# fallenshock/SinDDM

Hardware: AMD Instinct MI355X
Metric: diffusion steps/sec (finest scale) + imgs/sec full multi-scale sample, 1/2/4/8 GPU (higher is better)
Workload: dtype f32 (3x3 convs: binary16 hi/lo split products -- Winograd-domain GEMMs with all 4 MFMA terms, fp32 accumulate; fp32-equivalent, error vs float64 = the fp32 oracle's: tests/test_gpu_h2.py; everything else fp32); 1 GPU; C3: 6-scale pyramid, T=1000, finest scale 411x512, batch 64 per GPU, dim=160; batch_per_gpu=64, global_batch=64, scale=5, parallelism=independent chains over 1 GPU(s), one all-gather of the images

## Files before the change

### include/sinddm_hip_debug.h

```cpp
#ifndef SINDDM_HIP_DEBUG_H
#define SINDDM_HIP_DEBUG_H

#include <stddef.h>
#include <stdint.h>

#ifdef __cplusplus
extern "C" {
#endif

int sinddm_prof_begin(void);
int sinddm_prof_end(double* conv_ms_total, int64_t* conv_launches, double* conv_flops_total);
int sinddm_prof_end2(double* conv_ms_total, int64_t* conv_launches, double* conv_flops_total,
                     double* conv_exec_flops_total);
int sinddm_prof_end3(int kind, double* ms_total, int64_t* launches, double* flops_total,
                     double* exec_flops_total, int reset);

int sinddm_debug_conv_path(int dim, int B, int H, int W);

int sinddm_debug_infer_path(int dim, int B, int H, int W);

int sinddm_debug_train_path(int dim, int B, int H, int W);

int sinddm_debug_block_train(const float* params, const float* packed, const float* packed_bwd, int dim, int l,
                             const float* x, const float* cond_bias, const float* grad_y, float* y, float* grad_x,
                             float* grad_params, float* dcond, int B, int H, int W, void* ws, size_t ws_bytes,
                             void* stream);

int sinddm_debug_wgrad_map(int Cin, int Cout, int64_t ntiles, int ncu, uint32_t* wg_out, int wg_cap, int32_t* splits_out,
                           int splits_cap);

#ifdef __cplusplus
}
#endif
#endif
```

### sinddm_amd/_lib.py

```python
from __future__ import annotations

import ctypes as C
import os
from typing import Optional

import torch

_HERE = os.path.dirname(os.path.abspath(__file__))
LIB_PATH = os.path.join(_HERE, "libsinddm_hip.so")

ABI_SYMBOLS = (
    "sinddm_abi_version", "sinddm_param_count", "sinddm_param_tensors", "sinddm_param_offset",
    "sinddm_packed_count", "sinddm_workspace_bytes", "sinddm_pack_weights", "sinddm_net_forward",
    "sinddm_q_sample", "sinddm_reverse_step", "sinddm_reverse_step_edit", "sinddm_upsample_bilinear", "sinddm_prof_begin", "sinddm_prof_end", "sinddm_prof_end2", "sinddm_prof_end3", "sinddm_debug_wgrad_map", "sinddm_debug_conv_path",
    "sinddm_debug_block_train", "sinddm_debug_infer_path", "sinddm_debug_train_path",
    "sinddm_train_workspace_bytes", "sinddm_packed_bwd_count", "sinddm_pack_weights_bwd",
    "sinddm_net_forward_train", "sinddm_net_backward", "sinddm_l1_loss_fwd_bwd", "sinddm_adam_ema_step",
    "sinddm_cond_embed", "sinddm_cond_stride", "sinddm_sample_chain", "sinddm_sample_chain2", "sinddm_sample_chain_ex",
    "sinddm_normal_fill", "sinddm_wrap_halo", "sinddm_upsample_bilinear_wrap", "sinddm_sample_chain_tile",
    "sinddm_sample_chain_keep", "sinddm_reverse_step_keep", "sinddm_normal_fill_samples", "sinddm_sample_chain_seeds",
)


ABI_VERSION = 3
DIM_FP32_CONVS = 0x10000
TILE_HALO = 16


class StepCoefs(C.Structure):
    _fields_ = [("mode", C.c_int), ("clip", C.c_int),
                ("sqrt_recip_ac_t", C.c_float), ("sqrt_recipm1_ac_t", C.c_float),
                ("coef1_t", C.c_float), ("coef2_t", C.c_float),
                ("gamma_t", C.c_float), ("gamma_tm1", C.c_float),
                ("sqrt_ac_tm1", C.c_float), ("sqrt_ac_t", C.c_float), ("sqrt_1m_ac_t", C.c_float),
                ("sqrt_1m_ac_tm1_mvar", C.c_float), ("sigma", C.c_float)]


class ChainOpts(C.Structure):
    _fields_ = [("edit_w", C.c_void_p), ("edit_c", C.c_void_p), ("noise", C.c_void_p)]


class KeepOpts(C.Structure):
    _fields_ = [("mask", C.c_void_p), ("x0", C.c_void_p), ("ab", C.POINTER(C.c_float))]


class SinddmError(RuntimeError):
    pass


_lib: Optional[C.CDLL] = None


def load() -> C.CDLL:
# ... 19 lines not shown
        "sinddm_param_tensors": (i, [i]),
        "sinddm_param_offset": (i64, [i, i]),
        "sinddm_packed_count": (i64, [i]),
        "sinddm_workspace_bytes": (sz, [i, i, i, i]),
        "sinddm_pack_weights": (i, [p, p, i, p]),
        "sinddm_net_forward": (i, [p, p, p, p, i, f, p, i, i, i, i, p, sz, p]),
        "sinddm_cond_embed": (i, [p, p, i, f, i, i, p, p, p, p]),
        "sinddm_cond_stride": (i, [i]),
        "sinddm_q_sample": (i, [p, p, p, p, p, p, p, p, i, i, i64, p]),
        "sinddm_reverse_step": (i, [p, p, p, p, p, C.POINTER(StepCoefs), i64, p]),
        "sinddm_reverse_step_edit": (i, [p, p, p, p, p, C.POINTER(StepCoefs), p, p, i, i, i, p]),
        "sinddm_sample_chain": (i, chain[:-2] + [C.POINTER(C.c_int)]),
        "sinddm_sample_chain2": (i, chain),
        "sinddm_sample_chain_ex": (i, chain + [C.POINTER(ChainOpts)]),
        "sinddm_sample_chain_tile": (i, chain + [C.POINTER(ChainOpts), i, i]),
        "sinddm_sample_chain_keep": (i, chain + [C.POINTER(ChainOpts), i, i, C.POINTER(KeepOpts)]),
        "sinddm_sample_chain_seeds": (i, chain + [C.POINTER(ChainOpts), i, i, C.POINTER(KeepOpts), p]),
        "sinddm_normal_fill_samples": (i, [p, i, i64, p, C.c_uint64, p]),
        "sinddm_reverse_step_keep": (i, [p, p, p, p, p, C.POINTER(StepCoefs), p, p, p, p, f, f, i, i, i, p]),
        "sinddm_wrap_halo": (i, [p, p, i, i, i, i, i, p]),
        "sinddm_upsample_bilinear_wrap": (i, [p, p, i, i, i, i, i, i, i, p]),
        "sinddm_normal_fill": (i, [p, i64, C.c_uint64, C.c_uint64, p]),
        "sinddm_upsample_bilinear": (i, [p, p, i, i, i, i, i, p]),
        "sinddm_prof_begin": (i, []),
        "sinddm_prof_end": (i, [C.POINTER(C.c_double), C.POINTER(C.c_int64), C.POINTER(C.c_double)]),
        "sinddm_prof_end2": (i, [C.POINTER(C.c_double), C.POINTER(C.c_int64), C.POINTER(C.c_double),
                                 C.POINTER(C.c_double)]),
        "sinddm_prof_end3": (i, [i, C.POINTER(C.c_double), C.POINTER(C.c_int64), C.POINTER(C.c_double),
                                 C.POINTER(C.c_double), i]),
        "sinddm_debug_wgrad_map": (i, [i, i, i64, i, C.POINTER(C.c_uint32), i, C.POINTER(C.c_int32), i]),
        "sinddm_debug_conv_path": (i, [i, i, i, i]),
        "sinddm_debug_infer_path": (i, [i, i, i, i]),
        "sinddm_debug_train_path": (i, [i, i, i, i]),
        "sinddm_debug_block_train": (i, [p, p, p, i, i, p, p, p, p, p, p, p, i, i, i, p, sz, p]),
        "sinddm_train_workspace_bytes": (sz, [i, i, i, i]),
        "sinddm_packed_bwd_count": (i64, [i]),
        "sinddm_pack_weights_bwd": (i, [p, p, i, p]),
        "sinddm_net_forward_train": (i, [p, p, p, p, i, f, p, i, i, i, i, p, sz, p]),
        "sinddm_net_backward": (i, [p, p, p, p, p, p, p, i, i, i, i, p, sz, p]),
        "sinddm_l1_loss_fwd_bwd": (i, [p, p, p, p, i64, f, p]),
        "sinddm_adam_ema_step": (i, [p, p, p, p, p, f, f, f, f, f, f, f, i, i64, p]),
    }
    for name, (res, args) in sig.items():
        if not hasattr(lib, name):
            continue
        fn = getattr(lib, name)
        fn.restype = res
        fn.argtypes = args
    _lib = lib
    return lib


def missing_symbols():
    lib = load()
    return [s for s in ABI_SYMBOLS if not hasattr(lib, s)]


def check(rc: int, what: str) -> None:
    if rc != 0:
        kind = {-1: "bad argument", -2: "unsupported shape", -3: "workspace too small"}.get(rc, f"hipError {rc}")
        raise SinddmError(f"{what} failed: {kind}")


def ptr(t: Optional[torch.Tensor]) -> Optional[int]:
    if t is None:
        return None
# ... 10 lines not shown
```

### sinddm_amd/csrc/internal.h

```cpp
#pragma once
#include "common.h"

namespace sinddm {

struct PackSeg {
    long long dst;
    long long count;
    long long w;
    long long w2;
    int kind;
    int cin, cout, taps, nch, mt, co_lds;
    int transpose;
};
struct PackArgs {
    PackSeg seg[32];
    int nseg;
    long long total;
};
int pack_launch(const float* params, float* packed, const PackArgs& a, hipStream_t st);

struct TrainBufs {
    float* cond;
    float* emb;
    float* hpre;
    float* cvec;
    float* mvec;
    float* h[4];
    float* u[4];
    float* g[4];
    float* o[4];
    float* s[4];
    float* dcond;
    float* small;
    float* wscr;
    float* amax;
};

struct ChainStep;
int net_forward_impl(const NetPlan& P, const float* params, const float* packed, const float* x, const int64_t* t_dev,
                     int t_host, float scale, float* out, int B, int H, int W, void* ws, size_t ws_bytes,
                     hipStream_t st, const TrainBufs* tb, const ChainStep* cs = nullptr);

int block_forward(const NetPlan& P, int l, const float* params, const float* packed, const float* cur, const float* cond,
                  int cond_stride, float* hbuf, float* gbuf, float* obuf, float* upre, int B, int H, int W, hipStream_t st,
                  int Wt = 0, float* amax = nullptr);
int conv3x3_path(int cout, int cin, int coblks, int B, int H, int W);

struct ConvArgs;
bool wh_applies(const NetPlan& P, int B, int H, int W, int cin, int cout);
bool wh_enabled();
int wh_conv(const ConvArgs& c, hipStream_t st);
int wh_pack(const float* w, float* wsinv, void* img, int cin, int cout, int transpose, hipStream_t st);
int amax_tensor_launch(const float* x, float* amax, int B, long long per_sample, hipStream_t st);

int dwconv_launch(const float* x, const float* w, const float* bias, const float* cond, int cond_stride,
                  const float* addt, int flip, float* out, int B, int C, int H, int W, hipStream_t st, int pi = 0, int po = 0,
                  float* amax = nullptr);

}
```

### sinddm_amd/csrc/plan.h

```cpp
#pragma once
#include <stdint.h>

namespace sinddm {

constexpr int KC = 8;
constexpr int TIME_DIM = 32;
constexpr int CHANNELS = 3;

inline bool wh_plan_ok(int cin, int cout) { return cin >= 32 && cin % 16 == 0 && cout % 80 == 0; }
inline long long wh_plan_halfs(int cin, int cout) { return (long long)(cout / 80) * (cin / 16) * 24 * 5 * 512; }

struct BlockPlan {
    int cin, cout;
    int64_t mlp_w, mlp_b, tr_w, tr_b, dw_w, dw_b, c1_w, c1_b, c2_w, c2_b, res_w, res_b;
    int mt;
    int coblks;
    int co_lds;
    int nch1;
    int nch2;
    int nchr;
    int64_t pk_c1, pk_c2, pk_res, pk_b1, pk_b2;
    int nchw1, nchw2;
    int64_t pk_wc1, pk_wc2;
    int64_t pk_w1f, pk_w2f;
    int64_t pk_q1, pk_q2, pk_qs1, pk_qs2;
    int cond_off;
};

struct NetPlan {
    int dim, half;
    BlockPlan blk[4];
    int64_t tm0_w, tm0_b, tm2_w, tm2_b, fin_w, fin_b;
    int64_t nparams, npacked;
    int64_t pk_zero;
    int ntensors;
    int64_t tensor_off[64];
    int cond_stride;
    bool fp32_convs;
    bool ok;
};

inline int mt_for(int cout) { return (cout % 80 == 0) ? 5 : ((cout % 32 == 0) ? 2 : 1); }
inline int co_lds_for(int mt) { int m = mt * 16; return (m % 32 == 16) ? m : m + 16; }

inline NetPlan make_plan(int dim_arg) {
    NetPlan p{};
    const int dim = dim_arg & 0xFFFF;
    p.fp32_convs = (dim_arg & 0x10000) != 0;
    if (dim_arg < 0 || (dim_arg >> 17) != 0) { p.ok = false; return p; }
    p.ok = dim >= 2 && dim % 2 == 0 && dim <= 1024;
    p.dim = dim;
    p.half = dim / 2;
    int64_t o = 0;
    int nt = 0;
    auto take = [&](int64_t n) { int64_t r = o; p.tensor_off[nt++] = r; o += n; return r; };
    p.tm0_w = take(TIME_DIM * 4 * TIME_DIM * 2);
    p.tm0_b = take(TIME_DIM * 4);
    p.tm2_w = take(TIME_DIM * TIME_DIM * 4);
    p.tm2_b = take(TIME_DIM);
    const int cins[4] = {CHANNELS, p.half, dim, dim};
    const int couts[4] = {p.half, dim, dim, p.half};
    int64_t q = 0;
    int coff = 0;
    for (int l = 0; l < 4; ++l) {
        BlockPlan& b = p.blk[l];
        b.cin = cins[l];
        b.cout = couts[l];
// ... 18 lines not shown
        b.co_lds = co_lds_for(b.mt);
        b.nch1 = (b.cin + KC - 1) / KC;
        b.nch2 = (b.cout + KC - 1) / KC;
        b.nchr = (b.res_w >= 0) ? (b.cin + KC - 1) / KC : 0;
        b.pk_c1 = q; q += (int64_t)b.coblks * b.nch1 * 9 * KC * b.co_lds;
        b.pk_c2 = q; q += (int64_t)b.coblks * b.nch2 * 9 * KC * b.co_lds;
        b.pk_res = q; q += (int64_t)b.coblks * b.nchr * KC * b.co_lds;
        b.pk_b1 = q; q += (int64_t)b.coblks * b.mt * 16;
        b.pk_b2 = q; q += (int64_t)b.coblks * b.mt * 16;
        b.nchw1 = (b.cin + 15) / 16;
        b.nchw2 = (b.cout + 15) / 16;
        if (b.cin >= 8) { b.pk_wc1 = q; q += (int64_t)b.coblks * b.nchw1 * 16 * 4 * b.mt * 64; } else b.pk_wc1 = -1;
        b.pk_wc2 = q; q += (int64_t)b.coblks * b.nchw2 * 16 * 4 * b.mt * 64;
        const bool f24 = b.mt == 5 && b.cout % 80 == 0;
        if (f24 && b.cin >= 16 && b.cin % 16 == 0) { b.pk_w1f = q; q += (int64_t)b.coblks * b.nchw1 * 32768; } else b.pk_w1f = -1;
        if (f24 && b.cout % 16 == 0) { b.pk_w2f = q; q += (int64_t)b.coblks * b.nchw2 * 32768; } else b.pk_w2f = -1;
        q = (q + 63) / 64 * 64;
        if (wh_plan_ok(b.cin, b.cout)) {
            b.pk_q1 = q; q += wh_plan_halfs(b.cin, b.cout) / 2;
            b.pk_qs1 = q; q += (b.cout + 63) / 64 * 64;
        } else b.pk_q1 = b.pk_qs1 = -1;
        if (wh_plan_ok(b.cout, b.cout)) {
            b.pk_q2 = q; q += wh_plan_halfs(b.cout, b.cout) / 2;
            b.pk_qs2 = q; q += (b.cout + 63) / 64 * 64;
        } else b.pk_q2 = b.pk_qs2 = -1;
        b.cond_off = coff;
        coff += b.cin;
    }
    p.fin_w = take((int64_t)CHANNELS * p.half);
    p.fin_b = take(CHANNELS);
    p.nparams = o;
    p.pk_zero = q;
    q += 64;
    p.npacked = q;
    p.ntensors = nt;
    p.cond_stride = (coff + 3) / 4 * 4;
    return p;
}

}
```

### sinddm_amd/csrc/sinddm_fwd.hip

```cpp
#include "conv_mfma.h"
#include "conv_wino.h"
#include "conv_wino4.h"
#include "conv_wh.h"
#include "internal.h"
#include "step_tail.h"
#include <type_traits>
namespace sinddm {

ConvProfiler& conv_profiler() {
    static ConvProfiler p;
    return p;
}

__global__ void pack_kernel(const float* __restrict__ params, float* __restrict__ packed, PackArgs a) {
    long long i = (long long)blockIdx.x * blockDim.x + threadIdx.x;
    if (i >= a.total) return;
    int s = 0;
    long long base = 0;
    while (s < a.nseg - 1 && i >= base + a.seg[s].count) { base += a.seg[s].count; ++s; }
    const PackSeg& g = a.seg[s];
    const long long j = i - base;
    float v = 0.0f;
    if (g.kind == 0) {
        const int co_l = (int)(j % g.co_lds);
// ... 154 lines not shown
    auto addf = [&](PackSeg sg) { f.seg[n++] = sg; total += sg.count; };
    for (int l = 0; l < 4; ++l) {
        const BlockPlan& b = P.blk[l];
        PackSeg wz{};
        wz.kind = 4; wz.mt = b.mt; wz.transpose = 0; wz.w2 = -1; wz.taps = 9;
        if (b.pk_w1f >= 0) {
            wz.dst = b.pk_w1f; wz.nch = b.nchw1; wz.count = (long long)b.coblks * b.nchw1 * 32768;
            wz.w = b.c1_w; wz.cin = b.cin; wz.cout = b.cout;
            addf(wz);
        }
        if (b.pk_w2f >= 0) {
            wz.dst = b.pk_w2f; wz.nch = b.nchw2; wz.count = (long long)b.coblks * b.nchw2 * 32768;
            wz.w = b.c2_w; wz.cin = b.cout; wz.cout = b.cout;
            addf(wz);
        }
    }
    if (n > 0) {
        f.nseg = n;
        f.total = total;
        rc = pack_launch(params, packed, f, st);
        if (rc) return rc;
    }
    for (int l = 0; l < 4; ++l) {
        const BlockPlan& b = P.blk[l];
        if (b.pk_q1 >= 0) {
            rc = wh_pack_launch(params + b.c1_w, packed + b.pk_qs1, packed + b.pk_q1, b.cin, b.cout, 0, st);
            if (rc) return rc;
        }
        if (b.pk_q2 >= 0) {
            rc = wh_pack_launch(params + b.c2_w, packed + b.pk_qs2, packed + b.pk_q2, b.cout, b.cout, 0, st);
            if (rc) return rc;
        }
    }
    return 0;
}

struct CondArgs {
    const float* params;
    const long long* t_dev;
    int t_host;
    int t_step;
    float scale;
    float* out;
    int cond_stride;
    long long tm0_w, tm0_b, tm2_w, tm2_b;
    long long mlp_w[4], mlp_b[4], tr_w[4], tr_b[4];
    int cin[4], coff[4];
    float* cond_vec;
    float* hidden;
    float* emb_out;
    float* mvec_out;
};
static CondArgs cond_args(const NetPlan& P, const float* params) {
    CondArgs ca{};
    ca.params = params; ca.cond_stride = P.cond_stride;
    ca.tm0_w = P.tm0_w; ca.tm0_b = P.tm0_b; ca.tm2_w = P.tm2_w; ca.tm2_b = P.tm2_b;
    for (int l = 0; l < 4; ++l) {
        ca.mlp_w[l] = P.blk[l].mlp_w; ca.mlp_b[l] = P.blk[l].mlp_b;
        ca.tr_w[l] = P.blk[l].tr_w; ca.tr_b[l] = P.blk[l].tr_b;
        ca.cin[l] = P.blk[l].cin; ca.coff[l] = P.blk[l].cond_off;
    }
    return ca;
}

__global__ __launch_bounds__(128) void cond_kernel(CondArgs a) {
    __shared__ float emb[64];
    __shared__ float h1[128];
// ... 526 lines not shown
    for (int l = 0; l < 4; ++l) {
        const BlockPlan& b = P.blk[l];
        if (b.cout % 4 != 0) return false;
        if (b.cin != 3 && !(b.pk_wc1 >= 0 && b.cin % 4 == 0)) return false;
    }
    return true;
}
static int fwd_pitch(const NetPlan& P, int W) { return (W % 4 != 0 && plan_pads_rows(P)) ? (W + 3) / 4 * 4 : W; }
static size_t fwd_xpad_bytes(const NetPlan& P, int B, int H, int W) {
    return fwd_pitch(P, W) != W ? align_up((size_t)B * CHANNELS * H * fwd_pitch(P, W) * sizeof(float), 256) : 0;
}
static size_t fwd_workspace_core(const NetPlan& P, int B, int H, int W) {
    const size_t act = align_up((size_t)B * P.dim * H * fwd_pitch(P, W) * sizeof(float), 256);
    return cond_region_bytes(P, B) + 4 * act + fwd_xpad_bytes(P, B, H, W);
}
static size_t fwd_workspace_bytes(const NetPlan& P, int B, int H, int W) {
    return fwd_workspace_core(P, B, H, W) + 2 * cond_region_bytes(P, (B + 1) / 2) + 4096;
}

struct ChainStep {
    const float* cond_row;
    const float* x_tilde;
    float* x_next;
    TailArgs tail;
};

template <class F>
static void tail_dispatch(const TailArgs& t, F&& f) {
    auto keep = [&](auto e, auto n) { t.km ? f(e, n, std::true_type{}) : f(e, n, std::false_type{}); };
    auto noise = [&](auto e) { t.nz ? keep(e, std::true_type{}) : keep(e, std::false_type{}); };
    t.ew ? noise(std::true_type{}) : noise(std::false_type{});
}

int conv3x3_path(int cout, int cin, int coblks, int B, int H, int W) {
    if (!wino_enabled() || cout % 4 != 0) return 0;
    const bool f24 = mt_for(cout) == 5 && cout % 80 == 0 && cin >= 16 && cin % 16 == 0;
    const bool v3 = SINDDM_WINO_V3 && f24 &&
                    (long long)B * ((W + 31) / 32) * ((H + 3) / 4) * coblks >= SINDDM_V3_MIN_ITEMS_PER_CU * wino2_cu_count();
    if (v3 && SINDDM_WINO_V4 && conv_wino4_applies(B, H, W, coblks)) return 4;
    return v3 ? 3 : 2;
}

int block_forward(const NetPlan& P, int l, const float* params, const float* packed, const float* cur, const float* cond,
                  int cond_stride, float* hbuf, float* gbuf, float* obuf, float* upre, int B, int H, int W, hipStream_t st,
                  int Wt, float* amax) {
    const BlockPlan& b = P.blk[l];
    const bool wha = amax && b.pk_q1 >= 0 && conv_wh_applies(P.fp32_convs, B, H, W, b.cin, b.cout);
    const bool whb = amax && b.pk_q2 >= 0 && conv_wh_applies(P.fp32_convs, B, H, W, b.cout, b.cout);
    int rc = Wt > 0 ? dwconv_launch(cur, params + b.dw_w, params + b.dw_b, cond, cond_stride, nullptr, 0, hbuf, B, b.cin, H,
                                    Wt, st, W, W, wha ? amax : nullptr)
                    : dwconv_launch(cur, params + b.dw_w, params + b.dw_b, cond, cond_stride, nullptr, 0, hbuf, B, b.cin, H,
                                    W, st, 0, 0, wha ? amax : nullptr);
    if (rc) return rc;
    const bool wino = wino_enabled();
    ConvArgs c1{};
    c1.in = hbuf; c1.bias = packed + b.pk_b1; c1.out = gbuf;
    c1.B = B; c1.H = H; c1.W = W; c1.Cin = b.cin; c1.Cout = b.cout; c1.nch1 = 0;
    c1.coblks = b.coblks; c1.act = 1; c1.zero = packed + P.pk_zero; c1.Wt = Wt;
    c1.out_pre = upre;
    constexpr int c3 = SINDDM_CONV_C3;
    const bool v3 = SINDDM_WINO_V3 && wino &&
                    (long long)B * ((W + 31) / 32) * ((H + 3) / 4) * b.coblks >= SINDDM_V3_MIN_ITEMS_PER_CU * wino2_cu_count();
    const bool v4 = SINDDM_WINO_V4 && v3 && conv_wino4_applies(B, H, W, b.coblks);
    if (wha) {
        c1.w3 = packed + b.pk_q1; c1.wsinv = packed + b.pk_qs1; c1.amax_in = amax; c1.amax_out = whb ? amax + 1 : nullptr;
        c1.bias = params + b.c1_b;
        rc = conv_wh_launch(c1, st);
    } else if (v3 && b.pk_w1f >= 0) {
        c1.w3 = packed + b.pk_w1f; c1.nch3 = b.nchw1;
        rc = v4 ? conv_wino4_launch(c1, st) : conv_wino3_launch(c1, st);
    } else if (wino && b.pk_wc1 >= 0 && b.cin % 4 == 0) {
        c1.w3 = packed + b.pk_wc1; c1.nch3 = b.nchw1;
        rc = conv_wino_launch(c1, b.mt, st);
    } else if (b.cin == 3 && c3) {
        const int nwg = ((H * W + 255) / 256) * B;
        int split = 1;
        while (split < 8 && nwg * split < 2048 && b.cout % (split * 2) == 0) split *= 2;
        hipLaunchKernelGGL(conv3x3_c3_gelu_kernel, dim3((H * W + 255) / 256, B, split), dim3(256), 0, st, hbuf,
                           params + b.c1_w, params + b.c1_b, gbuf, c1.out_pre, H, W, b.cout, b.cout / split, Wt > 0 ? Wt : W,
                           whb ? amax + 1 : nullptr);
        SINDDM_LAUNCH_CHECK();
        rc = 0;
    } else {
        c1.w3 = packed + b.pk_c1; c1.nch3 = b.nch1;
        rc = conv_launch(c1, b.mt, st);
    }
    if (rc) return rc;
    if (whb && !(wha || (b.cin == 3 && c3 && !(v3 && b.pk_w1f >= 0) && !(wino && b.pk_wc1 >= 0 && b.cin % 4 == 0)))) {
        rc = amax_tensor_launch(gbuf, amax + 1, B, (long long)b.cout * H * W, st);
        if (rc) return rc;
    }
    ConvArgs c2{};
    c2.in = gbuf; c2.out = obuf;
    c2.B = B; c2.H = H; c2.W = W; c2.Cin = b.cout; c2.Cout = b.cout;
    c2.coblks = b.coblks; c2.act = 0; c2.zero = packed + P.pk_zero; c2.Wt = Wt;
    if (wino && b.cout % 4 == 0) {
        if (b.nchr > 0) {
            ConvArgs r1{};
            r1.in2 = cur; r1.Cin2 = b.cin; r1.w1 = packed + b.pk_res; r1.nch1 = b.nchr; r1.nch3 = 0;
            r1.bias = packed + b.pk_b2; r1.out = obuf; r1.Cout = b.cout; r1.coblks = b.coblks;
            r1.B = B; r1.H = H; r1.W = W; r1.zero = packed + P.pk_zero;
            rc = conv1x1_launch(r1, b.mt, st);
            if (rc) return rc;
            c2.resid = obuf; c2.bias = nullptr;
        } else {
            c2.resid = cur; c2.bias = packed + b.pk_b2;
        }
        c2.nch1 = 0;
        if (whb) {
            c2.w3 = packed + b.pk_q2; c2.wsinv = packed + b.pk_qs2; c2.amax_in = amax + 1;
            rc = conv_wh_launch(c2, st);
        } else if (v3 && b.pk_w2f >= 0) {
            c2.w3 = packed + b.pk_w2f; c2.nch3 = b.nchw2;
            rc = v4 ? conv_wino4_launch(c2, st) : conv_wino3_launch(c2, st);
        } else {
            c2.w3 = packed + b.pk_wc2; c2.nch3 = b.nchw2;
            rc = conv_wino_launch(c2, b.mt, st);
        }
    } else {
        c2.w3 = packed + b.pk_c2; c2.bias = packed + b.pk_b2; c2.nch3 = b.nch2;
// ... 37 lines not shown
                     int t_host, float scale, float* out, int B, int H, int W, void* ws, size_t ws_bytes,
                     hipStream_t st, const TrainBufs* tb, const ChainStep* cs) {
    FwdBuffers fb{};
    float* xpad = nullptr;
    float* amax = nullptr;
    if (tb) {
        fb.cond = tb->cond;
        amax = tb->amax;
    } else {
        if (ws_bytes < fwd_workspace_core(P, B, H, W)) return SINDDM_E_WORKSPACE;
        char* base = static_cast<char*>(ws);
        fb.cond = reinterpret_cast<float*>(base);
        base += cond_region_bytes(P, B);
        amax = reinterpret_cast<float*>(base - amax_region_bytes(B));
        const size_t act = align_up((size_t)B * P.dim * H * fwd_pitch(P, W) * sizeof(float), 256);
        for (int i = 0; i < 4; ++i) fb.buf[i] = reinterpret_cast<float*>(base + i * act);
        xpad = reinterpret_cast<float*>(base + 4 * act);
    }
    const int Wp = tb ? W : fwd_pitch(P, W);
    const bool padded = Wp != W;
    int cond_stride = P.cond_stride;
    if (cs) { fb.cond = const_cast<float*>(cs->cond_row); cond_stride = 0; }

    CondArgs ca = cond_args(P, params);
    ca.t_dev = reinterpret_cast<const long long*>(t_dev); ca.t_host = t_host; ca.scale = scale;
    ca.out = fb.cond;
    ca.cond_vec = tb ? tb->cvec : nullptr; ca.hidden = tb ? tb->hpre : nullptr;
    ca.emb_out = tb ? tb->emb : nullptr; ca.mvec_out = tb ? tb->mvec : nullptr;
    if (!cs) {
        hipLaunchKernelGGL(cond_kernel, dim3(B), dim3(128), 0, st, ca);
        SINDDM_LAUNCH_CHECK();
    }

    if (amax) {
        bool any = false;
        for (int l = 0; l < 4; ++l) {
            const BlockPlan& b = P.blk[l];
            any = any || (b.pk_q1 >= 0 && conv_wh_applies(P.fp32_convs, B, H, Wp, b.cin, b.cout)) ||
                  (b.pk_q2 >= 0 && conv_wh_applies(P.fp32_convs, B, H, Wp, b.cout, b.cout));
        }
        if (!any) amax = nullptr;
        else if (hipMemsetAsync(amax, 0, (size_t)B * AMAX_STRIDE * sizeof(float), st) != hipSuccess) return SINDDM_E_BADARG;
    }
    const float* cur = x;
    if (padded) {
        const long long nrows = (long long)B * CHANNELS * H;
        const long long nq = nrows * (Wp / 4);
        hipLaunchKernelGGL(pad_rows_kernel, dim3((unsigned)((nq + 255) / 256)), dim3(256), 0, st, x, xpad, H, W, Wp, nrows);
        SINDDM_LAUNCH_CHECK();
        cur = xpad;
    }
    int freeb[4] = {0, 1, 2, 3};
    int curb = -1;
    for (int l = 0; l < 4; ++l) {
        const BlockPlan& b = P.blk[l];
        int sel[3], n = 0;
        for (int i = 0; i < 4 && n < 3; ++i)
            if (freeb[i] != curb) sel[n++] = freeb[i];
        float* hbuf = tb ? tb->h[l] : fb.buf[sel[0]];
        float* gbuf = tb ? tb->g[l] : fb.buf[sel[1]];
        float* obuf = tb ? tb->o[l] : fb.buf[sel[2]];
        const int rc = block_forward(P, l, params, packed, cur, fb.cond + b.cond_off, cond_stride, hbuf, gbuf, obuf,
                                     tb ? tb->u[l] : nullptr, B, H, Wp, st, padded ? W : 0, amax ? amax + 2 * l : nullptr);
        if (rc) return rc;
        cur = obuf;
        curb = sel[2];
    }
    const int HW = H * W;
    if (padded) {
        const unsigned gx = (unsigned)((H * (Wp / 4) + 255) / 256);
        if (cs && cs->x_next)
            tail_dispatch(cs->tail, [&](auto E, auto N, auto K) {
                hipLaunchKernelGGL((final_conv_reverse_step_pitch_kernel<decltype(E)::value, decltype(N)::value, decltype(K)::value>),
                                   dim3(gx, B), dim3(256), 0, st, cur, params + P.fin_w, params + P.fin_b, x, cs->x_tilde,
                                   cs->x_next, P.half, H, W, Wp, cs->tail);
            });
        else
            hipLaunchKernelGGL(final_conv1x1_pitch_kernel, dim3(gx, B), dim3(256), 0, st, cur, params + P.fin_w,
                               params + P.fin_b, out, P.half, H, W, Wp);
        SINDDM_LAUNCH_CHECK();
        return 0;
    }
    if (cs && cs->x_next && HW % 4 == 0) {
        tail_dispatch(cs->tail, [&](auto E, auto N, auto K) {
            hipLaunchKernelGGL((final_conv_reverse_step_kernel<decltype(E)::value, decltype(N)::value, decltype(K)::value>),
                               dim3((HW / 4 + 255) / 256, B), dim3(256), 0, st, cur, params + P.fin_w, params + P.fin_b, x,
                               cs->x_tilde, cs->x_next, P.half, HW, cs->tail);
        });
        SINDDM_LAUNCH_CHECK();
        return 0;
    }
    hipLaunchKernelGGL(final_conv1x1_kernel, dim3(((HW + 3) / 4 + 255) / 256, B), dim3(256), 0, st, cur, params + P.fin_w,
                       params + P.fin_b, out, P.half, HW);
    SINDDM_LAUNCH_CHECK();
    return 0;
}

}

using namespace sinddm;

extern "C" {

int sinddm_abi_version(void) { return SINDDM_ABI_VERSION; }

int64_t sinddm_param_count(int dim) { NetPlan p = make_plan(dim); return p.ok ? p.nparams : -1; }
int sinddm_param_tensors(int dim) { NetPlan p = make_plan(dim); return p.ok ? p.ntensors : -1; }
int64_t sinddm_param_offset(int dim, int idx) {
    NetPlan p = make_plan(dim);
    if (!p.ok || idx < 0 || idx >= p.ntensors) return -1;
    return p.tensor_off[idx];
}
int64_t sinddm_packed_count(int dim) { NetPlan p = make_plan(dim); return p.ok ? p.npacked : -1; }

size_t sinddm_workspace_bytes(int dim, int B, int H, int W) {
    NetPlan p = make_plan(dim);
    if (!p.ok || B <= 0 || H <= 0 || W <= 0) return 0;
    return fwd_workspace_bytes(p, B, H, W);
}

// ... 349 lines not shown
#ifdef SINDDM_WINO_TIMING
int sinddm_debug_wino_timing(unsigned long long* host_dst, int n) {
    return (int)hipMemcpyFromSymbol(host_dst, HIP_SYMBOL(g_wino_dbg), sizeof(unsigned long long) * n);
}
#endif

int sinddm_prof_begin(void) {
    ConvProfiler& p = conv_profiler();
    p.on = true;
    p.used = 0;
    p.flops = 0.0;
    p.exec_flops = 0.0;
    return 0;
}

int sinddm_prof_end(double* conv_ms_total, int64_t* conv_launches, double* conv_flops_total) {
    return sinddm_prof_end2(conv_ms_total, conv_launches, conv_flops_total, nullptr);
}

int sinddm_prof_end2(double* conv_ms_total, int64_t* conv_launches, double* conv_flops_total,
                     double* conv_exec_flops_total) {
    return sinddm_prof_end3(0, conv_ms_total, conv_launches, conv_flops_total, conv_exec_flops_total, 1);
}

int sinddm_debug_infer_path(int dim, int B, int H, int W) {
    NetPlan p = make_plan(dim);
    if (!p.ok || B <= 0 || H <= 0 || W <= 0) return SINDDM_E_BADARG;
    const BlockPlan& b = p.blk[2];
    const int Wp = fwd_pitch(p, W);
    if (b.pk_q2 >= 0 && conv_wh_applies(p.fp32_convs, B, H, Wp, b.cout, b.cout)) return 8;
    return conv3x3_path(b.cout, b.cout, b.coblks, B, H, Wp);
}

int sinddm_prof_end3(int kind, double* ms_total, int64_t* launches, double* flops_total, double* exec_flops_total,
                     int reset) {
    ConvProfiler& p = conv_profiler();
    p.on = false;
    double ms = 0.0, fl = 0.0, ex = 0.0;
    int64_t n = 0;
    for (int i = 0; i < p.used; ++i) {
        if (kind >= 10 ? (p.kind[i] != kind / 10 || p.gen[i] != kind % 10) : (kind != 0 && p.kind[i] != kind)) continue;
        hipError_t e = hipEventSynchronize(p.ev[2 * i + 1]);
        if (e != hipSuccess) return (int)e;
        float t = 0.f;
        e = hipEventElapsedTime(&t, p.ev[2 * i], p.ev[2 * i + 1]);
        if (e != hipSuccess) return (int)e;
        ms += t; fl += p.rec_flops[i]; ex += p.rec_exec[i]; ++n;
    }
    if (ms_total) *ms_total = ms;
    if (launches) *launches = n;
    if (flops_total) *flops_total = fl;
    if (exec_flops_total) *exec_flops_total = ex;
    if (reset) { p.used = 0; p.flops = 0.0; p.exec_flops = 0.0; }
    return 0;
}

int sinddm_upsample_bilinear(const float* in, float* out, int BC, int h, int w, int H, int W, void* stream) {
    if (!in || !out || BC <= 0 || h <= 0 || w <= 0 || H <= 0 || W <= 0) return SINDDM_E_BADARG;
    const float sy = (float)h / (float)H, sx = (float)w / (float)W;
    hipLaunchKernelGGL((upsample_bilinear_kernel<false, false>), dim3((H * W + 255) / 256, BC), dim3(256), 0,
                       static_cast<hipStream_t>(stream), in, out, h, w, H, W, sy, sx);
    SINDDM_LAUNCH_CHECK();
    return 0;
}

int sinddm_upsample_bilinear_wrap(const float* in, float* out, int BC, int h, int w, int H, int W, int wrap_y, int wrap_x,
// ... 21 lines not shown
```

### sinddm_amd/csrc/step_tail.h

```cpp
#pragma once
#include "common.h"

namespace sinddm {

struct TailArgs {
    sinddm_step_coefs k;
    int b0;
    unsigned long long seed, step;
    const unsigned long long* sseeds;
    const float* ew;
    const float* ec;
    const float* nz;
    const float* km;
    const float* kx;
    float ka, kb;
};

__device__ __forceinline__ float reverse_step_mean(const sinddm_step_coefs& k, float x, float e, float xb, float w, float c,
                                                   bool edit) {
    float x0 = k.sqrt_recip_ac_t * x - k.sqrt_recipm1_ac_t * e;
    if (k.mode == 0) {
        if (edit) x0 = w * x0 + c;
        const float x0c = k.clip ? fminf(fmaxf(x0, -1.0f), 1.0f) : x0;
        return k.coef1_t * x0c + k.coef2_t * x;
    }
    float xp = (x0 - k.gamma_t * xb) / (1.0f - k.gamma_t);
    if (edit) xp = w * xp + c;
    if (k.mode == 1) {
        float mix = k.gamma_tm1 * xb + (1.0f - k.gamma_tm1) * xp;
        float x0c = x0;
        if (k.clip) {
            mix = fminf(fmaxf(mix, -1.0f), 1.0f);
            x0c = fminf(fmaxf(x0, -1.0f), 1.0f);
        }
// ... 109 lines not shown
                const float xb = a.k.mode != 0 ? xtil[i0 + j] : 0.f;
                out[i0 + j] = tail_eval<EDIT, KEEP>(a, xt[i0 + j], eps[i0 + j], xb, z[j], w[j], c[j], m[j], k0[j]);
            }
            continue;
        }
        f32x4 x{0.f, 0.f, 0.f, 0.f}, e{0.f, 0.f, 0.f, 0.f}, xb{0.f, 0.f, 0.f, 0.f};
        if (vec) {
            x = *reinterpret_cast<const f32x4*>(xt + i0);
            e = *reinterpret_cast<const f32x4*>(eps + i0);
            if (a.k.mode != 0) xb = *reinterpret_cast<const f32x4*>(xtil + i0);
        } else {
#pragma unroll
            for (int j = 0; j < 4; ++j) {
                if (j < nv) {
                    x[j] = xt[i0 + j];
                    e[j] = eps[i0 + j];
                    if (a.k.mode != 0) xb[j] = xtil[i0 + j];
                }
            }
        }
        f32x4 o;
#pragma unroll
        for (int j = 0; j < 4; ++j) o[j] = tail_eval<EDIT, KEEP>(a, x[j], e[j], xb[j], z[j], w[j], c[j], m[j], k0[j]);
        if (vec) {
            *reinterpret_cast<f32x4*>(out + i0) = o;
        } else {
#pragma unroll
            for (int j = 0; j < 4; ++j)
                if (j < nv) out[i0 + j] = o[j];
        }
    }
}

template <bool EDIT, bool NOISE, bool KEEP>
__global__ __launch_bounds__(256) void final_conv_reverse_step_kernel(const float* __restrict__ a, const float* __restrict__ w,
                                                                      const float* __restrict__ bias,
                                                                      const float* __restrict__ xt,
                                                                      const float* __restrict__ xtil, float* __restrict__ out,
                                                                      int C, int HW, TailArgs t) {
    const int b = blockIdx.y;
    const int p = (blockIdx.x * 256 + threadIdx.x) * 4;
    if (p >= HW) return;
    const NoiseKey nk = noise_key(t, b, (long long)3 * HW);
    const float* src = a + (size_t)b * C * HW + p;
    f32x4 e[3] = {{bias[0], bias[0], bias[0], bias[0]}, {bias[1], bias[1], bias[1], bias[1]}, {bias[2], bias[2], bias[2], bias[2]}};
#pragma unroll 8
    for (int c = 0; c < C; ++c) {
        const f32x4 v = *reinterpret_cast<const f32x4*>(src + (size_t)c * HW);
        e[0] += w[c] * v;
        e[1] += w[C + c] * v;
        e[2] += w[2 * C + c] * v;
    }
    f32x4 mw{1.f, 1.f, 1.f, 1.f};
    if (EDIT) mw = *reinterpret_cast<const f32x4*>(t.ew + p);
    f32x4 mk{0.f, 0.f, 0.f, 0.f};
    if (KEEP) mk = *reinterpret_cast<const f32x4*>(t.km + p);
#pragma unroll
    for (int c = 0; c < 3; ++c) {
        const long long i0 = ((long long)b * 3 + c) * HW + p;
        const long long ig = i0 + (long long)t.b0 * 3 * HW;
        float z[4] = {0.f, 0.f, 0.f, 0.f};
        if (tail_draws<KEEP>(t)) quad_draw<NOISE>(t.nz + ig, true, 4, nk.key, t.step, (unsigned long long)((i0 + nk.ofs) >> 2), z);
        const f32x4 x = *reinterpret_cast<const f32x4*>(xt + i0);
        f32x4 xb{0.f, 0.f, 0.f, 0.f};
        if (t.k.mode != 0) xb = *reinterpret_cast<const f32x4*>(xtil + i0);
        f32x4 mc{0.f, 0.f, 0.f, 0.f};
        if (EDIT) mc = *reinterpret_cast<const f32x4*>(t.ec + (size_t)c * HW + p);
        f32x4 o;
#pragma unroll
        for (int j = 0; j < 4; ++j) o[j] = tail_eval<EDIT, false>(t, x[j], e[c][j], xb[j], z[j], mw[j], mc[j], 0.f, 0.f);
        if (KEEP) {
            const f32x4 k0 = *reinterpret_cast<const f32x4*>(t.kx + (size_t)c * HW + p);
#pragma unroll
            for (int j = 0; j < 4; ++j) o[j] = keep_blend(t.k, o[j], z[j], xb[j], mk[j], k0[j], t.ka, t.kb);
        }
        *reinterpret_cast<f32x4*>(out + i0) = o;
    }
}

template <bool EDIT, bool NOISE, bool KEEP>
__global__ __launch_bounds__(256) void final_conv_reverse_step_pitch_kernel(
    const float* __restrict__ a, const float* __restrict__ w, const float* __restrict__ bias, const float* __restrict__ xt,
    const float* __restrict__ xtil, float* __restrict__ out, int C, int H, int W, int Wp, TailArgs t) {
    const int b = blockIdx.y;
    const int qpr = Wp >> 2;
    const int q = blockIdx.x * 256 + threadIdx.x;
    if (q >= H * qpr) return;
    const int y = q / qpr, x = (q - y * qpr) * 4;
    const size_t HWp = (size_t)H * Wp;
    const long long HW = (long long)H * W;
    const NoiseKey nk = noise_key(t, b, 3 * HW);
    const float* src = a + (size_t)b * C * HWp + (size_t)y * Wp + x;
    f32x4 e[3] = {{bias[0], bias[0], bias[0], bias[0]}, {bias[1], bias[1], bias[1], bias[1]}, {bias[2], bias[2], bias[2], bias[2]}};
#pragma unroll 8
    for (int c = 0; c < C; ++c) {
        const f32x4 v = *reinterpret_cast<const f32x4*>(src + (size_t)c * HWp);
        e[0] += w[c] * v;
        e[1] += w[C + c] * v;
        e[2] += w[2 * C + c] * v;
    }
    const int nv = W - x;
    const bool draw = tail_draws<KEEP>(t);
#pragma unroll
    for (int c = 0; c < 3; ++c) {
        const long long i0 = ((long long)b * 3 + c) * HW + (long long)y * W + x;
        const long long ig = i0 + (long long)t.b0 * 3 * HW;
        const long long ik = i0 + nk.ofs;
        const int r0 = (int)(ik & 3);
        float za[4] = {0.f, 0.f, 0.f, 0.f}, zb[4] = {0.f, 0.f, 0.f, 0.f};
        if (!NOISE && draw) {
            philox_normal4(nk.key, t.step, (unsigned long long)(ik >> 2), za);
            if (r0 != 0) philox_normal4(nk.key, t.step, (unsigned long long)(ik >> 2) + 1ull, zb);
        }
        const float z8[8] = {za[0], za[1], za[2], za[3], zb[0], zb[1], zb[2], zb[3]};
#pragma unroll
        for (int j = 0; j < 4; ++j) {
            if (j < nv) {
                float z = z8[j];
                z = r0 == 1 ? z8[j + 1] : z;
                z = r0 == 2 ? z8[j + 2] : z;
                z = r0 == 3 ? z8[j + 3] : z;
                if (NOISE) z = draw ? t.nz[ig + j] : 0.f;
                const int pp = y * W + x + j;
                const float xb = t.k.mode != 0 ? xtil[i0 + j] : 0.f;
                float mw = 1.f, mc = 0.f;
                if (EDIT) {
                    mw = t.ew[pp];
                    mc = t.ec[(size_t)c * HW + pp];
                }
                const float o = tail_eval<EDIT, false>(t, xt[i0 + j], e[c][j], xb, z, mw, mc, 0.f, 0.f);
                out[i0 + j] = KEEP ? keep_blend(t.k, o, z, xb, t.km[pp], t.kx[(size_t)c * HW + pp], t.ka, t.kb) : o;
            }
        }
// ... 18 lines not shown
```

Measured before the change: 718.3 sample-steps/s (finest scale, batch x steps/s, all GPUs).

## Collapse last block's second conv and residual into final 1x1 head

Because the final 1x1 conv is linear, the change precomposes it with the last block's 3x3 conv2 and residual 1x1 conv, giving a 3-output-channel 3x3 conv over the half-channel hidden map plus a 3-output 1x1 over the block input. The large half-by-half 3x3 conv (Winograd MFMA) and the writing and re-reading of the block output are skipped at inference, and a scalar FMA head kernel fused into the reverse-step tail computes eps directly. The composed weights are built in double precision at pack time. Rounding changes slightly, and the head kernel is a plain FMA loop that re-reads neighbour pixels through buffer loads.

```diff
diff --git a/include/sinddm_hip_debug.h b/include/sinddm_hip_debug.h
--- a/include/sinddm_hip_debug.h
+++ b/include/sinddm_hip_debug.h
@@ -19,6 +19,11 @@
 
 int sinddm_debug_infer_path(int dim, int B, int H, int W);
 
+int sinddm_debug_head_path(int dim, int B, int H, int W);
+int sinddm_debug_head_offsets(int dim, int64_t out[3]);
+int sinddm_debug_head(const float* packed, const float* g, const float* x_in, float* eps_out, int dim, int B, int H, int W,
+                      int Wp, void* stream);
+
 int sinddm_debug_train_path(int dim, int B, int H, int W);
 
 int sinddm_debug_block_train(const float* params, const float* packed, const float* packed_bwd, int dim, int l,
diff --git a/sinddm_amd/_lib.py b/sinddm_amd/_lib.py
--- a/sinddm_amd/_lib.py
+++ b/sinddm_amd/_lib.py
@@ -19,6 +19,7 @@
     "sinddm_cond_embed", "sinddm_cond_stride", "sinddm_sample_chain", "sinddm_sample_chain2", "sinddm_sample_chain_ex",
     "sinddm_normal_fill", "sinddm_wrap_halo", "sinddm_upsample_bilinear_wrap", "sinddm_sample_chain_tile",
     "sinddm_sample_chain_keep", "sinddm_reverse_step_keep", "sinddm_normal_fill_samples", "sinddm_sample_chain_seeds",
+    "sinddm_debug_head_path", "sinddm_debug_head_offsets", "sinddm_debug_head",
 )
 
 
@@ -104,6 +105,9 @@
         "sinddm_debug_conv_path": (i, [i, i, i, i]),
         "sinddm_debug_infer_path": (i, [i, i, i, i]),
         "sinddm_debug_train_path": (i, [i, i, i, i]),
+        "sinddm_debug_head_path": (i, [i, i, i, i]),
+        "sinddm_debug_head_offsets": (i, [i, C.POINTER(C.c_int64)]),
+        "sinddm_debug_head": (i, [p, p, p, p, i, i, i, i, i, p]),
         "sinddm_debug_block_train": (i, [p, p, p, i, i, p, p, p, p, p, p, p, i, i, i, p, sz, p]),
         "sinddm_train_workspace_bytes": (sz, [i, i, i, i]),
         "sinddm_packed_bwd_count": (i64, [i]),
diff --git a/sinddm_amd/csrc/head.h b/sinddm_amd/csrc/head.h
--- /dev/null
+++ b/sinddm_amd/csrc/head.h
@@ -0,0 +1,182 @@
+#pragma once
+#include "common.h"
+
+namespace sinddm {
+
+#ifndef SINDDM_HEAD_COLLAPSE
+#define SINDDM_HEAD_COLLAPSE 1
+#endif
+
+constexpr int HEAD_GROUP = 16;
+
+struct HeadPackArgs {
+    long long dst;
+    long long c2_w, c2_b, res_w, res_b;
+    long long fin_w, fin_b;
+    int half, dim;
+};
+__global__ __launch_bounds__(256) void head_pack_kernel(const float* __restrict__ params, float* __restrict__ packed,
+                                                        HeadPackArgs a) {
+    const int nc = a.half * CHANNELS * 9, nr = a.dim * CHANNELS;
+    const int i = blockIdx.x * 256 + threadIdx.x;
+    if (i >= nc + nr + CHANNELS) return;
+    const float* wf = params + a.fin_w;
+    double s = 0.;
+    if (i < nc) {
+        const int tap = i % 9, o = (i / 9) % CHANNELS, ci = i / (9 * CHANNELS);
+        for (int m = 0; m < a.half; ++m)
+            s += (double)wf[o * a.half + m] * (double)params[a.c2_w + ((long long)m * a.half + ci) * 9 + tap];
+    } else if (i < nc + nr) {
+        const int j = i - nc, o = j % CHANNELS, ci = j / CHANNELS;
+        for (int m = 0; m < a.half; ++m) s += (double)wf[o * a.half + m] * (double)params[a.res_w + (long long)m * a.dim + ci];
+    } else {
+        const int o = i - nc - nr;
+        for (int m = 0; m < a.half; ++m)
+            s += (double)wf[o * a.half + m] * ((double)params[a.c2_b + m] + (double)params[a.res_b + m]);
+        s += (double)params[a.fin_b + o];
+    }
+    packed[a.dst + i] = (float)s;
+}
+
+inline int head_pack_launch(const NetPlan& P, const float* params, float* packed, hipStream_t st) {
+    const BlockPlan& b = P.blk[3];
+    HeadPackArgs a{};
+    a.dst = P.pk_hc;
+    a.c2_w = b.c2_w; a.c2_b = b.c2_b; a.res_w = b.res_w; a.res_b = b.res_b;
+    a.fin_w = P.fin_w; a.fin_b = P.fin_b;
+    a.half = P.half; a.dim = P.dim;
+    const long long total = P.npacked - P.pk_hc;
+    hipLaunchKernelGGL(head_pack_kernel, dim3((unsigned)((total + 255) / 256)), dim3(256), 0, st, params, packed, a);
+    SINDDM_LAUNCH_CHECK();
+    return 0;
+}
+
+struct HeadEps {
+    const float* g;
+    const float* xin;
+    const float* wc;
+    const float* wr;
+    const float* bc;
+    int half, dim, H, Wp;
+
+    __device__ __forceinline__ void operator()(int b, int q, f32x4 (&e)[3]) const {
+        const int qpr = Wp >> 2;
+        const int y = q / qpr, x = (q - y * qpr) * 4;
+        const int plane = H * Wp;
+        constexpr int OOBI = 0x40000000;
+        int oq[3], ol[3], orr[3];
+#pragma unroll
+        for (int r = 0; r < 3; ++r) {
+            const int gy = y + r - 1;
+            const bool ok = gy >= 0 && gy < H;
+            const int base = (gy * Wp + x) * 4;
+            oq[r] = ok ? base : OOBI;
+            ol[r] = (ok && x >= 4) ? base - 4 : OOBI;
+            orr[r] = (ok && x + 4 < Wp) ? base + 16 : OOBI;
+        }
+#pragma unroll
+        for (int o = 0; o < 3; ++o) e[o] = f32x4{bc[o], bc[o], bc[o], bc[o]};
+        const float* gb = g + (size_t)b * half * plane;
+        auto fetch = [&](int c, float (&v)[3][6]) __attribute__((always_inline)) {
+            const __amdgpu_buffer_rsrc_t rs =
+                __builtin_amdgcn_make_buffer_rsrc(const_cast<float*>(gb + (size_t)c * plane), 0, plane * 4, 0x00020000);
+#pragma unroll
+            for (int r = 0; r < 3; ++r) {
+                const f32x4 m = __builtin_bit_cast(f32x4, __builtin_amdgcn_raw_buffer_load_b128(rs, oq[r], 0, 0));
+                v[r][0] = __builtin_bit_cast(float, __builtin_amdgcn_raw_buffer_load_b32(rs, ol[r], 0, 0));
+                v[r][1] = m[0]; v[r][2] = m[1]; v[r][3] = m[2]; v[r][4] = m[3];
+                v[r][5] = __builtin_bit_cast(float, __builtin_amdgcn_raw_buffer_load_b32(rs, orr[r], 0, 0));
+            }
+        };
+        float in[3][6];
+        fetch(0, in);
+        f32x4 p[3] = {{0.f, 0.f, 0.f, 0.f}, {0.f, 0.f, 0.f, 0.f}, {0.f, 0.f, 0.f, 0.f}};
+        for (int c = 0; c < half; ++c) {
+            float nx[3][6];
+            fetch(c + 1 < half ? c + 1 : c, nx);
+            const float* wk = wc + c * 27;
+#pragma unroll
+            for (int r = 0; r < 3; ++r)
+#pragma unroll
+                for (int o = 0; o < 3; ++o)
+#pragma unroll
+                    for (int kx = 0; kx < 3; ++kx)
+#pragma unroll
+                        for (int j = 0; j < 4; ++j) p[o][j] = fmaf(wk[o * 9 + r * 3 + kx], in[r][j + kx], p[o][j]);
+            if ((c + 1) % HEAD_GROUP == 0 || c + 1 == half) {
+#pragma unroll
+                for (int o = 0; o < 3; ++o) {
+                    e[o] += p[o];
+                    p[o] = f32x4{0.f, 0.f, 0.f, 0.f};
+                }
+            }
+#pragma unroll
+            for (int r = 0; r < 3; ++r)
+#pragma unroll
+                for (int k = 0; k < 6; ++k) in[r][k] = nx[r][k];
+        }
+        const float* xb = xin + (size_t)b * dim * plane + (size_t)q * 4;
+        for (int c0 = 0; c0 < dim; c0 += HEAD_GROUP) {
+            const int c1 = c0 + HEAD_GROUP < dim ? c0 + HEAD_GROUP : dim;
+            f32x4 p[3] = {{0.f, 0.f, 0.f, 0.f}, {0.f, 0.f, 0.f, 0.f}, {0.f, 0.f, 0.f, 0.f}};
+#pragma unroll 8
+            for (int c = c0; c < c1; ++c) {
+                const f32x4 v = *reinterpret_cast<const f32x4*>(xb + (size_t)c * plane);
+#pragma unroll
+                for (int o = 0; o < 3; ++o)
+#pragma unroll
+                    for (int j = 0; j < 4; ++j) p[o][j] = fmaf(wr[c * 3 + o], v[j], p[o][j]);
+            }
+#pragma unroll
+            for (int o = 0; o < 3; ++o) e[o] += p[o];
+        }
+    }
+};
+
+struct FinalConvEps {
+    const float* a;
+    const float* w;
+    const float* bias;
+    int C;
+    size_t plane;
+
+    __device__ __forceinline__ void operator()(int b, int q, f32x4 (&e)[3]) const {
+        const float* src = a + (size_t)b * C * plane + (size_t)q * 4;
+#pragma unroll
+        for (int o = 0; o < 3; ++o) e[o] = f32x4{bias[o], bias[o], bias[o], bias[o]};
+#pragma unroll 8
+        for (int c = 0; c < C; ++c) {
+            const f32x4 v = *reinterpret_cast<const f32x4*>(src + (size_t)c * plane);
+            e[0] += w[c] * v;
+            e[1] += w[C + c] * v;
+            e[2] += w[2 * C + c] * v;
+        }
+    }
+};
+
+__global__ __launch_bounds__(256) void head_eps_kernel(HeadEps h, float* __restrict__ out, int W) {
+    const int b = blockIdx.y;
+    const int qpr = h.Wp >> 2;
+    const int q = blockIdx.x * 256 + threadIdx.x;
+    if (q >= h.H * qpr) return;
+    f32x4 e[3];
+    h(b, q, e);
+    const int y = q / qpr, x = (q - y * qpr) * 4;
+    const size_t HW = (size_t)h.H * W;
+    float* dst = out + (size_t)b * 3 * HW + (size_t)y * W + x;
+    if (W == h.Wp) {
+#pragma unroll
+        for (int c = 0; c < 3; ++c) *reinterpret_cast<f32x4*>(dst + c * HW) = e[c];
+    } else {
+#pragma unroll
+        for (int j = 0; j < 4; ++j) {
+            if (x + j < W) {
+                dst[j] = e[0][j];
+                dst[HW + j] = e[1][j];
+                dst[2 * HW + j] = e[2][j];
+            }
+        }
+    }
+}
+
+}
diff --git a/sinddm_amd/csrc/internal.h b/sinddm_amd/csrc/internal.h
--- a/sinddm_amd/csrc/internal.h
+++ b/sinddm_amd/csrc/internal.h
@@ -43,7 +43,7 @@
 
 int block_forward(const NetPlan& P, int l, const float* params, const float* packed, const float* cur, const float* cond,
                   int cond_stride, float* hbuf, float* gbuf, float* obuf, float* upre, int B, int H, int W, hipStream_t st,
-                  int Wt = 0, float* amax = nullptr);
+                  int Wt = 0, float* amax = nullptr, bool skip2 = false);
 int conv3x3_path(int cout, int cin, int coblks, int B, int H, int W);
 
 struct ConvArgs;
diff --git a/sinddm_amd/csrc/plan.h b/sinddm_amd/csrc/plan.h
--- a/sinddm_amd/csrc/plan.h
+++ b/sinddm_amd/csrc/plan.h
@@ -33,6 +33,7 @@
     int64_t tm0_w, tm0_b, tm2_w, tm2_b, fin_w, fin_b;
     int64_t nparams, npacked;
     int64_t pk_zero;
+    int64_t pk_hc, pk_hr, pk_hb;
     int ntensors;
     int64_t tensor_off[64];
     int cond_stride;
@@ -117,6 +118,9 @@
     p.nparams = o;
     p.pk_zero = q;
     q += 64;
+    p.pk_hc = q; q += (int64_t)p.half * CHANNELS * 9;
+    p.pk_hr = q; q += (int64_t)dim * CHANNELS;
+    p.pk_hb = q; q += CHANNELS;
     p.npacked = q;
     p.ntensors = nt;
     p.cond_stride = (coff + 3) / 4 * 4;
diff --git a/sinddm_amd/csrc/sinddm_fwd.hip b/sinddm_amd/csrc/sinddm_fwd.hip
--- a/sinddm_amd/csrc/sinddm_fwd.hip
+++ b/sinddm_amd/csrc/sinddm_fwd.hip
@@ -210,7 +210,7 @@
             if (rc) return rc;
         }
     }
-    return 0;
+    return head_pack_launch(P, params, packed, st);
 }
 
 struct CondArgs {
@@ -803,6 +803,13 @@
     t.ew ? noise(std::true_type{}) : noise(std::false_type{});
 }
 
+static bool head_applies(const TrainBufs* tb, int H, int Wp) {
+    return SINDDM_HEAD_COLLAPSE && !tb && Wp % 4 == 0 && (long long)H * Wp < (1LL << 28);
+}
+static HeadEps head_eps(const NetPlan& P, const float* packed, const float* g, const float* xin, int H, int Wp) {
+    return HeadEps{g, xin, packed + P.pk_hc, packed + P.pk_hr, packed + P.pk_hb, P.half, P.dim, H, Wp};
+}
+
 int conv3x3_path(int cout, int cin, int coblks, int B, int H, int W) {
     if (!wino_enabled() || cout % 4 != 0) return 0;
     const bool f24 = mt_for(cout) == 5 && cout % 80 == 0 && cin >= 16 && cin % 16 == 0;
@@ -814,10 +821,10 @@
 
 int block_forward(const NetPlan& P, int l, const float* params, const float* packed, const float* cur, const float* cond,
                   int cond_stride, float* hbuf, float* gbuf, float* obuf, float* upre, int B, int H, int W, hipStream_t st,
-                  int Wt, float* amax) {
+                  int Wt, float* amax, bool skip2) {
     const BlockPlan& b = P.blk[l];
     const bool wha = amax && b.pk_q1 >= 0 && conv_wh_applies(P.fp32_convs, B, H, W, b.cin, b.cout);
-    const bool whb = amax && b.pk_q2 >= 0 && conv_wh_applies(P.fp32_convs, B, H, W, b.cout, b.cout);
+    const bool whb = !skip2 && amax && b.pk_q2 >= 0 && conv_wh_applies(P.fp32_convs, B, H, W, b.cout, b.cout);
     int rc = Wt > 0 ? dwconv_launch(cur, params + b.dw_w, params + b.dw_b, cond, cond_stride, nullptr, 0, hbuf, B, b.cin, H,
                                     Wt, st, W, W, wha ? amax : nullptr)
                     : dwconv_launch(cur, params + b.dw_w, params + b.dw_b, cond, cond_stride, nullptr, 0, hbuf, B, b.cin, H,
@@ -856,7 +863,7 @@
         c1.w3 = packed + b.pk_c1; c1.nch3 = b.nch1;
         rc = conv_launch(c1, b.mt, st);
     }
-    if (rc) return rc;
+    if (rc || skip2) return rc;
     if (whb && !(wha || (b.cin == 3 && c3 && !(v3 && b.pk_w1f >= 0) && !(wino && b.pk_wc1 >= 0 && b.cin % 4 == 0)))) {
         rc = amax_tensor_launch(gbuf, amax + 1, B, (long long)b.cout * H * W, st);
         if (rc) return rc;
@@ -960,12 +967,13 @@
         SINDDM_LAUNCH_CHECK();
     }
 
+    const bool head = head_applies(tb, H, Wp);
     if (amax) {
         bool any = false;
         for (int l = 0; l < 4; ++l) {
             const BlockPlan& b = P.blk[l];
             any = any || (b.pk_q1 >= 0 && conv_wh_applies(P.fp32_convs, B, H, Wp, b.cin, b.cout)) ||
-                  (b.pk_q2 >= 0 && conv_wh_applies(P.fp32_convs, B, H, Wp, b.cout, b.cout));
+                  (!(head && l == 3) && b.pk_q2 >= 0 && conv_wh_applies(P.fp32_convs, B, H, Wp, b.cout, b.cout));
         }
         if (!any) amax = nullptr;
         else if (hipMemsetAsync(amax, 0, (size_t)B * AMAX_STRIDE * sizeof(float), st) != hipSuccess) return SINDDM_E_BADARG;
@@ -980,6 +988,7 @@
     }
     int freeb[4] = {0, 1, 2, 3};
     int curb = -1;
+    const float* head_g = nullptr;
     for (int l = 0; l < 4; ++l) {
         const BlockPlan& b = P.blk[l];
         int sel[3], n = 0;
@@ -988,20 +997,41 @@
         float* hbuf = tb ? tb->h[l] : fb.buf[sel[0]];
         float* gbuf = tb ? tb->g[l] : fb.buf[sel[1]];
         float* obuf = tb ? tb->o[l] : fb.buf[sel[2]];
+        const bool skip2 = head && l == 3;
         const int rc = block_forward(P, l, params, packed, cur, fb.cond + b.cond_off, cond_stride, hbuf, gbuf, obuf,
-                                     tb ? tb->u[l] : nullptr, B, H, Wp, st, padded ? W : 0, amax ? amax + 2 * l : nullptr);
+                                     tb ? tb->u[l] : nullptr, B, H, Wp, st, padded ? W : 0, amax ? amax + 2 * l : nullptr,
+                                     skip2);
         if (rc) return rc;
+        if (skip2) { head_g = gbuf; break; }
         cur = obuf;
         curb = sel[2];
     }
     const int HW = H * W;
+    if (head) {
+        const HeadEps he = head_eps(P, packed, head_g, cur, H, Wp);
+        const dim3 grid((unsigned)((H * (Wp / 4) + 255) / 256), B);
+        if (cs && cs->x_next && padded)
+            tail_dispatch(cs->tail, [&](auto E, auto N, auto K) {
+                hipLaunchKernelGGL((final_conv_reverse_step_pitch_kernel<decltype(E)::value, decltype(N)::value, decltype(K)::value, HeadEps>),
+                                   grid, dim3(256), 0, st, he, x, cs->x_tilde, cs->x_next, H, W, Wp, cs->tail);
+            });
+        else if (cs && cs->x_next)
+            tail_dispatch(cs->tail, [&](auto E, auto N, auto K) {
+                hipLaunchKernelGGL((final_conv_reverse_step_kernel<decltype(E)::value, decltype(N)::value, decltype(K)::value, HeadEps>),
+                                   grid, dim3(256), 0, st, he, x, cs->x_tilde, cs->x_next, HW, cs->tail);
+            });
+        else
+            hipLaunchKernelGGL(head_eps_kernel, grid, dim3(256), 0, st, he, out, W);
+        SINDDM_LAUNCH_CHECK();
+        return 0;
+    }
+    const FinalConvEps fe{cur, params + P.fin_w, params + P.fin_b, P.half, (size_t)H * Wp};
     if (padded) {
         const unsigned gx = (unsigned)((H * (Wp / 4) + 255) / 256);
         if (cs && cs->x_next)
             tail_dispatch(cs->tail, [&](auto E, auto N, auto K) {
-                hipLaunchKernelGGL((final_conv_reverse_step_pitch_kernel<decltype(E)::value, decltype(N)::value, decltype(K)::value>),
-                                   dim3(gx, B), dim3(256), 0, st, cur, params + P.fin_w, params + P.fin_b, x, cs->x_tilde,
-                                   cs->x_next, P.half, H, W, Wp, cs->tail);
+                hipLaunchKernelGGL((final_conv_reverse_step_pitch_kernel<decltype(E)::value, decltype(N)::value, decltype(K)::value, FinalConvEps>),
+                                   dim3(gx, B), dim3(256), 0, st, fe, x, cs->x_tilde, cs->x_next, H, W, Wp, cs->tail);
             });
         else
             hipLaunchKernelGGL(final_conv1x1_pitch_kernel, dim3(gx, B), dim3(256), 0, st, cur, params + P.fin_w,
@@ -1011,9 +1041,8 @@
     }
     if (cs && cs->x_next && HW % 4 == 0) {
         tail_dispatch(cs->tail, [&](auto E, auto N, auto K) {
-            hipLaunchKernelGGL((final_conv_reverse_step_kernel<decltype(E)::value, decltype(N)::value, decltype(K)::value>),
-                               dim3((HW / 4 + 255) / 256, B), dim3(256), 0, st, cur, params + P.fin_w, params + P.fin_b, x,
-                               cs->x_tilde, cs->x_next, P.half, HW, cs->tail);
+            hipLaunchKernelGGL((final_conv_reverse_step_kernel<decltype(E)::value, decltype(N)::value, decltype(K)::value, FinalConvEps>),
+                               dim3((HW / 4 + 255) / 256, B), dim3(256), 0, st, fe, x, cs->x_tilde, cs->x_next, HW, cs->tail);
         });
         SINDDM_LAUNCH_CHECK();
         return 0;
@@ -1429,6 +1458,31 @@
     return conv3x3_path(b.cout, b.cout, b.coblks, B, H, Wp);
 }
 
+int sinddm_debug_head_path(int dim, int B, int H, int W) {
+    NetPlan p = make_plan(dim);
+    if (!p.ok || B <= 0 || H <= 0 || W <= 0) return SINDDM_E_BADARG;
+    return head_applies(nullptr, H, fwd_pitch(p, W)) ? 1 : 0;
+}
+
+int sinddm_debug_head_offsets(int dim, int64_t out[3]) {
+    NetPlan p = make_plan(dim);
+    if (!p.ok || !out) return SINDDM_E_BADARG;
+    out[0] = p.pk_hc; out[1] = p.pk_hr; out[2] = p.pk_hb;
+    return 0;
+}
+
+int sinddm_debug_head(const float* packed, const float* g, const float* x_in, float* eps_out, int dim, int B, int H, int W,
+                      int Wp, void* stream) {
+    if (!packed || !g || !x_in || !eps_out || B <= 0 || H <= 0 || W <= 0) return SINDDM_E_BADARG;
+    NetPlan p = make_plan(dim);
+    if (!p.ok) return SINDDM_E_BADSHAPE;
+    if (Wp % 4 != 0 || W > Wp || W <= Wp - 4 || (long long)H * Wp >= (1LL << 28) || B > 65535) return SINDDM_E_BADSHAPE;
+    hipLaunchKernelGGL(head_eps_kernel, dim3((unsigned)((H * (Wp / 4) + 255) / 256), B), dim3(256), 0,
+                       static_cast<hipStream_t>(stream), head_eps(p, packed, g, x_in, H, Wp), eps_out, W);
+    SINDDM_LAUNCH_CHECK();
+    return 0;
+}
+
 int sinddm_prof_end3(int kind, double* ms_total, int64_t* launches, double* flops_total, double* exec_flops_total,
                      int reset) {
     ConvProfiler& p = conv_profiler();
diff --git a/sinddm_amd/csrc/step_tail.h b/sinddm_amd/csrc/step_tail.h
--- a/sinddm_amd/csrc/step_tail.h
+++ b/sinddm_amd/csrc/step_tail.h
@@ -1,5 +1,6 @@
 #pragma once
 #include "common.h"
+#include "head.h"
 
 namespace sinddm {
 
@@ -175,25 +176,16 @@
     }
 }
 
-template <bool EDIT, bool NOISE, bool KEEP>
-__global__ __launch_bounds__(256) void final_conv_reverse_step_kernel(const float* __restrict__ a, const float* __restrict__ w,
-                                                                      const float* __restrict__ bias,
-                                                                      const float* __restrict__ xt,
+template <bool EDIT, bool NOISE, bool KEEP, class EPS>
+__global__ __launch_bounds__(256) void final_conv_reverse_step_kernel(EPS eps, const float* __restrict__ xt,
                                                                       const float* __restrict__ xtil, float* __restrict__ out,
-                                                                      int C, int HW, TailArgs t) {
+                                                                      int HW, TailArgs t) {
     const int b = blockIdx.y;
     const int p = (blockIdx.x * 256 + threadIdx.x) * 4;
     if (p >= HW) return;
     const NoiseKey nk = noise_key(t, b, (long long)3 * HW);
-    const float* src = a + (size_t)b * C * HW + p;
-    f32x4 e[3] = {{bias[0], bias[0], bias[0], bias[0]}, {bias[1], bias[1], bias[1], bias[1]}, {bias[2], bias[2], bias[2], bias[2]}};
-#pragma unroll 8
-    for (int c = 0; c < C; ++c) {
-        const f32x4 v = *reinterpret_cast<const f32x4*>(src + (size_t)c * HW);
-        e[0] += w[c] * v;
-        e[1] += w[C + c] * v;
-        e[2] += w[2 * C + c] * v;
-    }
+    f32x4 e[3];
+    eps(b, p >> 2, e);
     f32x4 mw{1.f, 1.f, 1.f, 1.f};
     if (EDIT) mw = *reinterpret_cast<const f32x4*>(t.ew + p);
     f32x4 mk{0.f, 0.f, 0.f, 0.f};
@@ -221,27 +213,20 @@
     }
 }
 
-template <bool EDIT, bool NOISE, bool KEEP>
-__global__ __launch_bounds__(256) void final_conv_reverse_step_pitch_kernel(
-    const float* __restrict__ a, const float* __restrict__ w, const float* __restrict__ bias, const float* __restrict__ xt,
-    const float* __restrict__ xtil, float* __restrict__ out, int C, int H, int W, int Wp, TailArgs t) {
+template <bool EDIT, bool NOISE, bool KEEP, class EPS>
+__global__ __launch_bounds__(256) void final_conv_reverse_step_pitch_kernel(EPS eps, const float* __restrict__ xt,
+                                                                            const float* __restrict__ xtil,
+                                                                            float* __restrict__ out, int H, int W, int Wp,
+                                                                            TailArgs t) {
     const int b = blockIdx.y;
     const int qpr = Wp >> 2;
     const int q = blockIdx.x * 256 + threadIdx.x;
     if (q >= H * qpr) return;
     const int y = q / qpr, x = (q - y * qpr) * 4;
-    const size_t HWp = (size_t)H * Wp;
     const long long HW = (long long)H * W;
     const NoiseKey nk = noise_key(t, b, 3 * HW);
-    const float* src = a + (size_t)b * C * HWp + (size_t)y * Wp + x;
-    f32x4 e[3] = {{bias[0], bias[0], bias[0], bias[0]}, {bias[1], bias[1], bias[1], bias[1]}, {bias[2], bias[2], bias[2], bias[2]}};
-#pragma unroll 8
-    for (int c = 0; c < C; ++c) {
-        const f32x4 v = *reinterpret_cast<const f32x4*>(src + (size_t)c * HWp);
-        e[0] += w[c] * v;
-        e[1] += w[C + c] * v;
-        e[2] += w[2 * C + c] * v;
-    }
+    f32x4 e[3];
+    eps(b, q, e);
     const int nv = W - x;
     const bool draw = tail_draws<KEEP>(t);
 #pragma unroll
```

New measurement: 767.2 sample-steps/s (finest scale, batch x steps/s, all GPUs), median of 6. +6.8%, better.
